# BIGBALLON/distribuuuu

Hardware: AMD Instinct MI355X
Metric: images/sec resnet50 train (whole node) (higher is better)
Workload: dtype bf16; 1 GPU; model=resnet50, global_batch=256, im_size=224, parallelism=dp1, syncbn=False, hipgraph=True

## Files before the change

### distribuuuu_amd/csrc/bind.cpp

```cpp
#include <torch/extension.h>

at::Tensor relu_fwd(at::Tensor x);
at::Tensor relu_bwd(at::Tensor gy, at::Tensor y);
at::Tensor add_relu_fwd(at::Tensor a, at::Tensor b);
at::Tensor se_scale_fwd(at::Tensor x, at::Tensor s);
at::Tensor dropout_fwd(at::Tensor x, double p, int64_t seed);
std::vector<at::Tensor> se_scale_bwd(at::Tensor gy, at::Tensor x,
                                     at::Tensor s);
std::vector<at::Tensor> bn_sums(at::Tensor x);
at::Tensor bn_reduce_partials(at::Tensor part);
std::vector<at::Tensor> bn_stats(at::Tensor x, at::Tensor gamma,
                                 at::Tensor beta,
                                 c10::optional<at::Tensor> rm_opt,
                                 c10::optional<at::Tensor> rv_opt,
                                 double momentum, double eps, bool training,
                                 c10::optional<at::Tensor> part_opt);
at::Tensor bn_apply_act(at::Tensor x, at::Tensor scale, at::Tensor shift,
                        int64_t act, c10::optional<at::Tensor> res);
at::Tensor bn_bwd_stats(at::Tensor gy, at::Tensor x,
                        c10::optional<at::Tensor> res, at::Tensor scale,
                        at::Tensor shift, int64_t act);
std::vector<at::Tensor> bn_bwd_apply(at::Tensor gy, at::Tensor x,
                                     c10::optional<at::Tensor> res,
                                     at::Tensor mean, at::Tensor rstd,
                                     at::Tensor gamma, at::Tensor scale,
                                     at::Tensor shift, at::Tensor sums,
                                     double total_count, int64_t act,
                                     bool training, bool need_gres);
std::vector<at::Tensor> bn_bwd(at::Tensor gy, at::Tensor x,
                               c10::optional<at::Tensor> res, at::Tensor mean,
                               at::Tensor rstd, at::Tensor gamma,
                               at::Tensor scale, at::Tensor shift,
                               int64_t act, bool training, bool need_gres,
                               c10::optional<at::Tensor> mask);
std::vector<at::Tensor> bn_apply_act_mask(at::Tensor x, at::Tensor scale,
                                          at::Tensor shift, int64_t act,
                                          at::Tensor res);
at::Tensor bn_apply_act_pad(at::Tensor x, at::Tensor scale, at::Tensor shift,
                            int64_t act, int64_t ph, int64_t pw);
std::vector<at::Tensor> bn_bwd_pad(at::Tensor gy, at::Tensor x,
                                   at::Tensor mean, at::Tensor rstd,
                                   at::Tensor gamma, at::Tensor scale,
                                   at::Tensor shift, int64_t act,
                                   bool training, int64_t ph, int64_t pw);
std::vector<at::Tensor> maxpool_fwd(at::Tensor x, int64_t K, int64_t S,
                                    int64_t P);
at::Tensor maxpool_bwd(at::Tensor gy, at::Tensor idx, int64_t H, int64_t W,
                       int64_t K, int64_t S, int64_t P);
at::Tensor gap_fwd(at::Tensor x);
at::Tensor gap_bwd(at::Tensor gy, int64_t H, int64_t W);
at::Tensor avgpool_fwd(at::Tensor x, int64_t K, int64_t S);
at::Tensor avgpool_bwd(at::Tensor gy, int64_t K, int64_t S, int64_t H,
                       int64_t W);
std::vector<at::Tensor> ce_fwd(at::Tensor logits, at::Tensor target);
at::Tensor ce_bwd(at::Tensor logits, at::Tensor target, at::Tensor lse,
                  at::Tensor gl);
std::vector<at::Tensor> topk_acc(at::Tensor logits, at::Tensor target,
                                 int64_t topk);
at::Tensor conv2d_fwd_v1(at::Tensor x, at::Tensor w, at::Tensor y,
                         int64_t Ho, int64_t Wo, int64_t sh, int64_t sw,
                         int64_t ph, int64_t pw, int64_t dh, int64_t dw,
                         int64_t groups);
at::Tensor conv2d_fwd(at::Tensor x, at::Tensor w, int64_t sh, int64_t sw,
                      int64_t ph, int64_t pw, int64_t dh, int64_t dw,
                      int64_t groups);
std::vector<at::Tensor> conv2d_fwd_bn(at::Tensor x, at::Tensor w, int64_t sh,
                                      int64_t sw, int64_t ph, int64_t pw,
                                      int64_t dh, int64_t dw, int64_t groups);
at::Tensor conv2d_dgrad(at::Tensor gy, at::Tensor w, int64_t H, int64_t W,
                        int64_t sh, int64_t sw, int64_t ph, int64_t pw,
                        int64_t dh, int64_t dw, int64_t groups);
std::vector<at::Tensor> conv2d_dgrad_bn(at::Tensor gy, at::Tensor w,
                                        int64_t H, int64_t W, int64_t sh,
                                        int64_t sw, int64_t ph, int64_t pw,
                                        int64_t dh, int64_t dw,
                                        int64_t groups, at::Tensor bnx,
                                        at::Tensor bnscale, at::Tensor bnshift,
                                        int64_t bnact);

std::tuple<at::Tensor, int64_t> conv2d_dgrad_acc(
    at::Tensor gy, at::Tensor w, int64_t H, int64_t W, int64_t sh, int64_t sw,
    int64_t ph, int64_t pw, int64_t dh, int64_t dw, int64_t groups,
    at::Tensor into, c10::optional<at::Tensor> pre_opt, int64_t pre_kind);

std::vector<at::Tensor> conv2d_dgrad_prep(at::Tensor w, int64_t Kt0,
                                          int64_t sh, int64_t sw, int64_t ph,
                                          int64_t pw, int64_t dh, int64_t dw,
                                          int64_t groups);

at::Tensor conv2d_dgrad_pre(at::Tensor gy, at::Tensor w, int64_t H,
                            int64_t W, int64_t sh, int64_t sw, int64_t ph,
                            int64_t pw, int64_t dh, int64_t dw,
                            int64_t groups, at::Tensor pre,
                            int64_t pre_kind);
at::Tensor gemm_nt(at::Tensor a, at::Tensor b);
at::Tensor conv2d_fwd_v2(at::Tensor x, at::Tensor w, int64_t sh, int64_t sw,
                         int64_t ph, int64_t pw, int64_t dh, int64_t dw);
at::Tensor weight_flip_t(at::Tensor w, int64_t groups);
at::Tensor dilate_nhwc(at::Tensor x, int64_t sh, int64_t sw);
at::Tensor pad_channels(at::Tensor x, int64_t Cn);
at::Tensor conv2d_wgrad(at::Tensor gy, at::Tensor x, int64_t R, int64_t S,
                        int64_t sh, int64_t sw, int64_t ph, int64_t pw,
                        int64_t dh, int64_t dw, int64_t groups);
at::Tensor dwconv_fwd(at::Tensor x, at::Tensor w, int64_t sh, int64_t sw,
                      int64_t ph, int64_t pw);
at::Tensor dwconv_dgrad(at::Tensor gy, at::Tensor w, int64_t H, int64_t W,
                        int64_t sh, int64_t sw, int64_t ph, int64_t pw);
at::Tensor dwconv_wgrad(at::Tensor gy, at::Tensor x, int64_t R, int64_t S,
                        int64_t sh, int64_t sw, int64_t ph, int64_t pw);
at::Tensor mhsa_fwd(at::Tensor q, at::Tensor k, at::Tensor vt, at::Tensor rw,
                    at::Tensor rh, int64_t H, int64_t W,
                    c10::optional<at::Tensor> pout, int64_t heads,
                    int64_t qpix, int64_t kpix, double scale);
std::vector<at::Tensor> mhsa_bwd(at::Tensor dO, at::Tensor P, at::Tensor q,
                                 at::Tensor kt, at::Tensor v,
                                 at::Tensor rel_w, at::Tensor rel_h,
                                 int64_t H, int64_t W, int64_t heads,
                                 int64_t qpix, int64_t kqoff, int64_t vpix,
                                 int64_t opix, double scale,
                                 at::Tensor dqk_out, at::Tensor dv_out);
at::Tensor mhsa_rel_tables(at::Tensor q, at::Tensor rel, int64_t rows,
                           int64_t heads, int64_t L, int64_t qpix,
                           double scale);
at::Tensor aug_crop_flip_norm(at::Tensor raw, at::Tensor meta, int64_t S,
                              std::vector<double> mean,
                              std::vector<double> std, at::ScalarType dtype);
void set_deterministic(bool on);
bool is_deterministic();
void sgd_step(at::Tensor table, double lr, double momentum,
              double dampening, double weight_decay, bool nesterov);

PYBIND11_MODULE(TORCH_EXTENSION_NAME, m) {
  m.def("relu_fwd", &relu_fwd);
  m.def("relu_bwd", &relu_bwd);
  m.def("add_relu_fwd", &add_relu_fwd);
  m.def("se_scale_fwd", &se_scale_fwd);
  m.def("dropout_fwd", &dropout_fwd);
  m.def("se_scale_bwd", &se_scale_bwd);
  m.def("bn_sums", &bn_sums);
  m.def("bn_reduce_partials", &bn_reduce_partials);
  m.def("bn_stats", &bn_stats, py::arg("x"), py::arg("gamma"), py::arg("beta"),
        py::arg("rm") = py::none(), py::arg("rv") = py::none(),
        py::arg("momentum") = 0.1, py::arg("eps") = 1e-5,
        py::arg("training") = true, py::arg("part") = py::none());
  m.def("bn_apply_act", &bn_apply_act, py::arg("x"), py::arg("scale"),
        py::arg("shift"), py::arg("act"), py::arg("res") = py::none());
  m.def("bn_apply_act_mask", &bn_apply_act_mask);
  m.def("bn_apply_act_pad", &bn_apply_act_pad);
  m.def("bn_bwd_pad", &bn_bwd_pad);
  m.def("bn_bwd_stats", &bn_bwd_stats, py::arg("gy"), py::arg("x"),
        py::arg("res"), py::arg("scale"), py::arg("shift"),
        py::arg("act"));
  m.def("bn_bwd_apply", &bn_bwd_apply, py::arg("gy"), py::arg("x"),
        py::arg("res"), py::arg("mean"), py::arg("rstd"),
        py::arg("gamma"), py::arg("scale"), py::arg("shift"), py::arg("sums"),
        py::arg("total_count"), py::arg("act"), py::arg("training"),
        py::arg("need_gres"));
  m.def("bn_bwd", &bn_bwd, py::arg("gy"), py::arg("x"),
        py::arg("res"), py::arg("mean"), py::arg("rstd"), py::arg("gamma"),
        py::arg("scale"), py::arg("shift"), py::arg("act"),
        py::arg("training"), py::arg("need_gres"),
        py::arg("mask") = py::none());
  m.def("maxpool_fwd", &maxpool_fwd);
  m.def("maxpool_bwd", &maxpool_bwd);
  m.def("gap_fwd", &gap_fwd);
  m.def("gap_bwd", &gap_bwd);
  m.def("avgpool_fwd", &avgpool_fwd);
  m.def("avgpool_bwd", &avgpool_bwd);
  m.def("ce_fwd", &ce_fwd);
  m.def("ce_bwd", &ce_bwd);
  m.def("topk_acc", &topk_acc);
  m.def("sgd_step", &sgd_step);
  m.def("conv2d_fwd", &conv2d_fwd);
  m.def("conv2d_fwd_v1", &conv2d_fwd_v1);
  m.def("conv2d_fwd_bn", &conv2d_fwd_bn);
  m.def("conv2d_dgrad", &conv2d_dgrad);
  m.def("conv2d_dgrad_bn", &conv2d_dgrad_bn);
  m.def("conv2d_dgrad_acc", &conv2d_dgrad_acc);
  m.def("conv2d_dgrad_prep", &conv2d_dgrad_prep);
  m.def("conv2d_dgrad_pre", &conv2d_dgrad_pre);
  m.def("conv2d_wgrad", &conv2d_wgrad);
  m.def("gemm_nt", &gemm_nt);
  m.def("conv2d_fwd_v2", &conv2d_fwd_v2);
  m.def("weight_flip_t", &weight_flip_t);
  m.def("dilate_nhwc", &dilate_nhwc);
  m.def("pad_channels", &pad_channels);
  m.def("dwconv_fwd", &dwconv_fwd);
  m.def("dwconv_dgrad", &dwconv_dgrad);
  m.def("dwconv_wgrad", &dwconv_wgrad);
  m.def("mhsa_fwd", &mhsa_fwd);
  m.def("mhsa_bwd", &mhsa_bwd);
  m.def("mhsa_rel_tables", &mhsa_rel_tables);
  m.def("aug_crop_flip_norm", &aug_crop_flip_norm);
  m.def("set_deterministic", &set_deterministic);
  m.def("is_deterministic", &is_deterministic);
}
```

### distribuuuu_amd/csrc/conv.hip

```cpp
#include "common.h"

static int v2_minrsc() {
  static const int v = []() {
    const char* e = getenv("DISTRIBUUUU_V2_MINRSC");
    return e ? atoi(e) : 512;
  }();
  return v;
}

static int v2_into_minrsc() {
  static const int v = []() {
    const char* e = getenv("DISTRIBUUUU_V2INTO_MINRSC");
    return e ? atoi(e) : v2_minrsc();
  }();
  return v;
}


typedef __attribute__((ext_vector_type(8))) short short8;
typedef __attribute__((ext_vector_type(4))) float f32x4;
typedef __bf16 bf16x8 __attribute__((ext_vector_type(8)));

namespace {

// ... 461 lines not shown
  int C, H, W;
  int R, S, SC;
  int sh, sw, ph, pw;
  int Ho, Wo;
  int RSC, RSCp;
  int64_t M;
  unsigned long long magicHoWo, magicWo, magicSC, magicC;
  float* part;
};

DEV_INLINE int magic_div2(int m, unsigned long long magic) {
  return (int)(((unsigned long long)(unsigned)m * magic) >> 47);
}

template <bool EMIT>
__global__ __launch_bounds__(256) void conv_smallk_kernel(SmallConvParams p) {
  __shared__ float slab4[4][16 * 68];
  const int tid = threadIdx.x, lane = tid & 63, wid = tid >> 6;
  const int il = lane & 15, kq = lane >> 4;
  const int64_t mbase = (int64_t)blockIdx.x * 256 + wid * 64;
  int pn[4], prow[4], pcol[4];
  bool mok[4];
#pragma unroll
  for (int mi = 0; mi < 4; ++mi) {
    const int64_t m = mbase + mi * 16 + il;
    mok[mi] = m < p.M;
    const int mm = (int)(mok[mi] ? m : 0);
    const int n = magic_div2(mm, p.magicHoWo);
    const int rem = mm - n * (p.Ho * p.Wo);
    const int ho = magic_div2(rem, p.magicWo);
    const int wo = rem - ho * p.Wo;
    pn[mi] = n;
    prow[mi] = ho * p.sh - p.ph;
    pcol[mi] = wo * p.sw - p.pw;
  }
  const __hip_bfloat16* wr[4];
#pragma unroll
  for (int ni = 0; ni < 4; ++ni)
    wr[ni] = p.w + (int64_t)(ni * 16 + il) * p.RSCp + kq * 8;
  f32x4 acc[4][4] = {};
  if (p.C % 32 == 0) {
    const int csteps = p.C / 32;
    for (int r = 0; r < p.R; ++r) {
#pragma unroll 1
      for (int sidx = 0; sidx < p.S; ++sidx) {
        const __hip_bfloat16* ab[4];
        bool ok[4];
#pragma unroll
        for (int mi = 0; mi < 4; ++mi) {
          const int h = prow[mi] + r;
          const int w_ = pcol[mi] + sidx;
          ok[mi] = mok[mi] && h >= 0 && h < p.H && w_ >= 0 && w_ < p.W;
          ab[mi] = p.x +
                   (((int64_t)pn[mi] * p.H + h) * p.W + w_) * p.C + kq * 8;
        }
        const int e0 = (r * p.S + sidx) * p.C;
        for (int cc = 0; cc < csteps; ++cc) {
          bf16x8 afrag[4], bfrag[4];
#pragma unroll
          for (int mi = 0; mi < 4; ++mi)
            afrag[mi] = ok[mi] ? *reinterpret_cast<const bf16x8*>(ab[mi] +
                                                                  cc * 32)
                               : bf16x8{};
#pragma unroll
          for (int ni = 0; ni < 4; ++ni)
            bfrag[ni] =
                *reinterpret_cast<const bf16x8*>(wr[ni] + e0 + cc * 32);
#pragma unroll
          for (int mi = 0; mi < 4; ++mi)
#pragma unroll
            for (int ni = 0; ni < 4; ++ni)
              acc[mi][ni] = __builtin_amdgcn_mfma_f32_16x16x32_bf16(
                  afrag[mi], bfrag[ni], acc[mi][ni], 0, 0, 0);
        }
      }
    }
  } else {
    const int ksteps = p.RSCp / 32;
    for (int t = 0; t < ksteps; ++t) {
      const int e = t * 32 + kq * 8;
      const int r = magic_div2(e, p.magicSC);
      const int rem2 = e - r * p.SC;
      const int sidx = magic_div2(rem2, p.magicC);
      const int c = rem2 - sidx * p.C;
      bf16x8 afrag[4], bfrag[4];
#pragma unroll
      for (int mi = 0; mi < 4; ++mi) {
        const int h = prow[mi] + r;
        const int w_ = pcol[mi] + sidx;
        const bool ok = mok[mi] && e < p.RSC && h >= 0 && h < p.H &&
                        w_ >= 0 && w_ < p.W;
        afrag[mi] =
            ok ? *reinterpret_cast<const bf16x8*>(
                     p.x + (((int64_t)pn[mi] * p.H + h) * p.W + w_) * p.C + c)
               : bf16x8{};
      }
#pragma unroll
      for (int ni = 0; ni < 4; ++ni)
        bfrag[ni] = *reinterpret_cast<const bf16x8*>(wr[ni] + t * 32);
#pragma unroll
      for (int mi = 0; mi < 4; ++mi)
#pragma unroll
        for (int ni = 0; ni < 4; ++ni)
          acc[mi][ni] = __builtin_amdgcn_mfma_f32_16x16x32_bf16(
              afrag[mi], bfrag[ni], acc[mi][ni], 0, 0, 0);
    }
  }
  float* slab = slab4[wid];
  const int er = lane >> 2, ec = (lane & 3) << 4;
  float ps = 0.f, pq = 0.f;
#pragma unroll
  for (int mi = 0; mi < 4; ++mi) {
#pragma unroll
    for (int ni = 0; ni < 4; ++ni)
#pragma unroll
      for (int rr = 0; rr < 4; ++rr)
        slab[(kq * 4 + rr) * 68 + ni * 16 + il] = acc[mi][ni][rr];
    __builtin_amdgcn_wave_barrier();
    const int64_t m = mbase + mi * 16 + er;
    if (m < p.M) {
      union {
        __hip_bfloat16 b[16];
        uint4 q[2];
      } u;
#pragma unroll
      for (int j = 0; j < 16; ++j)
        u.b[j] = from_f32<__hip_bfloat16>(slab[er * 68 + ec + j]);
      __hip_bfloat16* yp = p.y + m * 64 + ec;
      *reinterpret_cast<uint4*>(yp) = u.q[0];
      *reinterpret_cast<uint4*>(yp + 8) = u.q[1];
    }
    if (EMIT)
      bn_partial_col_accum(slab, ps, pq,
                           (int)min((int64_t)16, p.M - (mbase + mi * 16)),
                           lane);
    __builtin_amdgcn_wave_barrier();
  }
  if (EMIT) {
    __shared__ float xarea[3][2][64];
    if (wid > 0) {
      xarea[wid - 1][0][lane] = ps;
      xarea[wid - 1][1][lane] = pq;
    }
    __syncthreads();
    if (wid == 0) {
#pragma unroll
      for (int j = 0; j < 3; ++j) {
        ps += xarea[j][0][lane];
        pq += xarea[j][1][lane];
      }
      bn_partial_store(p.part, (int64_t)blockIdx.x * 128, 64, lane, 64, ps,
                       pq);
    }
  }
}


template <int CSTEPS, bool EMIT>
__global__ __launch_bounds__(256) void conv_smallk_pipe_kernel(
    SmallConvParams p) {
  __shared__ float slab4[4][16 * 68];
  const int tid = threadIdx.x, lane = tid & 63, wid = tid >> 6;
  const int il = lane & 15, kq = lane >> 4;
  const int64_t mbase = (int64_t)blockIdx.x * 256 + wid * 64;
  int pn[4], prow[4], pcol[4];
  bool mok[4];
#pragma unroll
  for (int mi = 0; mi < 4; ++mi) {
    const int64_t m = mbase + mi * 16 + il;
    mok[mi] = m < p.M;
    const int mm = (int)(mok[mi] ? m : 0);
    const int n = magic_div2(mm, p.magicHoWo);
    const int rem = mm - n * (p.Ho * p.Wo);
    const int ho = magic_div2(rem, p.magicWo);
    const int wo = rem - ho * p.Wo;
    pn[mi] = n;
    prow[mi] = ho * p.sh - p.ph;
    pcol[mi] = wo * p.sw - p.pw;
  }
  const __hip_bfloat16* wr[4];
#pragma unroll
  for (int ni = 0; ni < 4; ++ni)
    wr[ni] = p.w + (int64_t)(ni * 16 + il) * p.RSCp + kq * 8;
  const int S = p.S;
  const int steps = p.R * S * CSTEPS;
  int r = 0, si = 0, cc = 0;
  bf16x8 Af[2][4], Bf[2][4];
  auto issue = [&](int buf) {
#pragma unroll
    for (int mi = 0; mi < 4; ++mi) {
      const int h = prow[mi] + r;
      const int w_ = pcol[mi] + si;
      const bool ok = mok[mi] && h >= 0 && h < p.H && w_ >= 0 && w_ < p.W;
      const __hip_bfloat16* ap =
          ok ? p.x + (((int64_t)pn[mi] * p.H + h) * p.W + w_) * p.C +
                   cc * 32 + kq * 8
             : p.zbuf;
      Af[buf][mi] = *reinterpret_cast<const bf16x8*>(ap);
    }
    const int e0 = (r * S + si) * p.C + cc * 32;
#pragma unroll
    for (int ni = 0; ni < 4; ++ni)
      Bf[buf][ni] = *reinterpret_cast<const bf16x8*>(wr[ni] + e0);
    ++cc;
    if (cc == CSTEPS) {
      cc = 0;
      ++si;
      if (si == S) {
        si = 0;
        ++r;
      }
    }
  };
  f32x4 acc[4][4] = {};
  issue(0);
  for (int i = 0; i < steps; i += 2) {
    if (i + 1 < steps) issue(1);
#pragma unroll
    for (int mi = 0; mi < 4; ++mi)
#pragma unroll
      for (int ni = 0; ni < 4; ++ni)
        acc[mi][ni] = __builtin_amdgcn_mfma_f32_16x16x32_bf16(
            Af[0][mi], Bf[0][ni], acc[mi][ni], 0, 0, 0);
    if (i + 1 < steps) {
      if (i + 2 < steps) issue(0);
#pragma unroll
      for (int mi = 0; mi < 4; ++mi)
#pragma unroll
        for (int ni = 0; ni < 4; ++ni)
          acc[mi][ni] = __builtin_amdgcn_mfma_f32_16x16x32_bf16(
              Af[1][mi], Bf[1][ni], acc[mi][ni], 0, 0, 0);
    }
  }
  float* slab = slab4[wid];
  const int er = lane >> 2, ec = (lane & 3) << 4;
  float ps = 0.f, pq = 0.f;
#pragma unroll
  for (int mi = 0; mi < 4; ++mi) {
#pragma unroll
    for (int ni = 0; ni < 4; ++ni)
#pragma unroll
      for (int rr = 0; rr < 4; ++rr)
        slab[(kq * 4 + rr) * 68 + ni * 16 + il] = acc[mi][ni][rr];
    __builtin_amdgcn_wave_barrier();
    const int64_t m = mbase + mi * 16 + er;
    if (m < p.M) {
      union {
        __hip_bfloat16 b[16];
        uint4 q[2];
      } u;
#pragma unroll
      for (int j = 0; j < 16; ++j)
        u.b[j] = from_f32<__hip_bfloat16>(slab[er * 68 + ec + j]);
      __hip_bfloat16* yp = p.y + m * 64 + ec;
      *reinterpret_cast<uint4*>(yp) = u.q[0];
      *reinterpret_cast<uint4*>(yp + 8) = u.q[1];
    }
    if (EMIT)
      bn_partial_col_accum(slab, ps, pq,
                           (int)min((int64_t)16, p.M - (mbase + mi * 16)),
                           lane);
    __builtin_amdgcn_wave_barrier();
  }
  if (EMIT) {
    __shared__ float xarea[3][2][64];
    if (wid > 0) {
      xarea[wid - 1][0][lane] = ps;
      xarea[wid - 1][1][lane] = pq;
    }
    __syncthreads();
    if (wid == 0) {
#pragma unroll
      for (int j = 0; j < 3; ++j) {
        ps += xarea[j][0][lane];
        pq += xarea[j][1][lane];
      }
      bn_partial_store(p.part, (int64_t)blockIdx.x * 128, 64, lane, 64, ps,
                       pq);
    }
  }
}

}

at::Tensor conv2d_fwd_into_fp32(at::Tensor x, at::Tensor w, at::Tensor y,
                                int64_t Ho, int64_t Wo, int64_t sh, int64_t sw,
                                int64_t ph, int64_t pw, int64_t dh, int64_t dw,
                                int64_t groups, int64_t osh, int64_t osw,
                                int64_t oh0, int64_t ow0,
                                at::Tensor* part_out);

struct BnBwdEmit {
  const __hip_bfloat16* x;
  const float* scale;
  const float* shift;
  int act;
};

at::Tensor conv2d_fwd_v2_into(at::Tensor x, at::Tensor w, at::Tensor y,
                              int64_t Ho, int64_t Wo, int64_t groups,
                              int64_t osh, int64_t osw, int64_t oh0,
                              int64_t ow0, bool acc = false);

at::Tensor conv2d_fwd_into(at::Tensor x, at::Tensor w, at::Tensor y, int64_t Ho,
                           int64_t Wo, int64_t sh, int64_t sw, int64_t ph,
                           int64_t pw, int64_t dh, int64_t dw, int64_t groups,
                           int64_t osh = 1, int64_t osw = 1, int64_t oh0 = 0,
                           int64_t ow0 = 0, at::Tensor* part_out = nullptr,
                           const BnBwdEmit* bemit = nullptr,
                           bool acc = false) {
  CHECK_GPU(x);
  if (x.scalar_type() == at::kFloat)
    return conv2d_fwd_into_fp32(x, w, y, Ho, Wo, sh, sw, ph, pw, dh, dw,
                                groups, osh, osw, oh0, ow0,
                                bemit ? nullptr : part_out);
  TORCH_CHECK(x.scalar_type() == at::kBFloat16, "conv2d_fwd: bf16/fp32 only");
  {
    static const bool v2i_off = []() {
      const char* e = getenv("DISTRIBUUUU_CONV_V2INTO");
      return e && e[0] == '0';
    }();
    const int Cgi = w.size(1), Ri = w.size(2), Si = w.size(3);
    const int Kgi = (int)(w.size(0) / groups);
    if (!v2i_off && part_out == nullptr && bemit == nullptr && ph == 0 &&
        pw == 0 && sh == 1 && sw == 1 && dh == 1 && dw == 1 &&
        (Si * Cgi) % 64 == 0 && Kgi >= 96 &&
        (int64_t)Ri * Si * Cgi >= v2_into_minrsc() && Cgi % 8 == 0 &&
        Ho + Ri - 1 <= x.size(2) && Wo + Si - 1 <= x.size(3))
      return conv2d_fwd_v2_into(x, w, y, Ho, Wo, groups, osh, osw, oh0, ow0,
                                acc);
  }
  check_nhwc(x, "x");
  check_nhwc(w, "w");
  const int N = x.size(0), Ct = x.size(1), H = x.size(2), W = x.size(3);
  const int Kt = w.size(0), Cg = w.size(1), R = w.size(2), S = w.size(3);
  TORCH_CHECK(Ct == Cg * groups, "channel/group mismatch");
  TORCH_CHECK(Cg % 8 == 0, "conv2d_fwd: per-group C must be a multiple of 8");
  const int Kg = Kt / groups;
  ConvParams p;
  p.x = (const __hip_bfloat16*)x.data_ptr();
  p.w = (const __hip_bfloat16*)w.data_ptr();
  p.y = (__hip_bfloat16*)y.data_ptr();
  p.N = N; p.H = H; p.W = W; p.Ct = Ct; p.Kt = Kt;
  p.R = R; p.S = S; p.Cg = Cg; p.Kg = Kg;
  p.sh = sh; p.sw = sw; p.ph = ph; p.pw = pw; p.dh = dh; p.dw = dw;
  p.Ho = Ho; p.Wo = Wo;
  p.HoA = y.size(2); p.WoA = y.size(3);
  p.osh = osh; p.osw = osw;
  p.oh0 = oh0; p.ow0 = ow0;
  p.M = N * Ho * Wo;
  p.nspan = (S * Cg + BK - 1) / BK;
  p.ksteps = R * p.nspan;
  p.tiles_m = (p.M + BM - 1) / BM;
  p.part = nullptr;
  p.bnx = nullptr;
  p.bnscale = nullptr;
  p.bnshift = nullptr;
  p.bnact = 0;
  dim3 grid(p.tiles_m, (Kg + BN - 1) / BN, groups);
  if (bemit != nullptr) {
    *part_out = at::empty({(int64_t)p.tiles_m, (int64_t)2 * Kt},
                          x.options().dtype(at::kFloat));
    p.part = part_out->data_ptr<float>();
    p.bnx = bemit->x;
    p.bnscale = bemit->scale;
    p.bnshift = bemit->shift;
    p.bnact = bemit->act;
    hipLaunchKernelGGL(conv_igemm_fwd_kernel<2>, grid, dim3(256), 0,
                       cur_stream(), p);
  } else if (part_out != nullptr) {
    *part_out = at::empty({(int64_t)p.tiles_m, (int64_t)2 * Kt},
                          x.options().dtype(at::kFloat));
    p.part = part_out->data_ptr<float>();
    hipLaunchKernelGGL(conv_igemm_fwd_kernel<1>, grid, dim3(256), 0,
                       cur_stream(), p);
  } else if (acc) {
    hipLaunchKernelGGL((conv_igemm_fwd_kernel<0, true>), grid, dim3(256), 0,
                       cur_stream(), p);
  } else {
    hipLaunchKernelGGL(conv_igemm_fwd_kernel<0>, grid, dim3(256), 0,
                       cur_stream(), p);
  }
  return y;
}

at::Tensor conv2d_fwd_v2p(at::Tensor x, at::Tensor w, int64_t sh, int64_t sw,
                          int64_t ph, int64_t pw, int64_t dh, int64_t dw,
                          int64_t groups, at::Tensor* part_out,
                          const BnBwdEmit* bemit = nullptr);
at::Tensor conv2d_fwd_v2_flat(at::Tensor x, at::Tensor wp, int64_t Kt_,
                              int64_t Cg_, int64_t R_, int64_t S_, int64_t sh,
                              int64_t sw, int64_t ph, int64_t pw, int64_t dh,
                              int64_t dw, int64_t groups,
                              at::Tensor* part_out, const BnBwdEmit* bemit,
                              at::Tensor* acc_into = nullptr);

static at::Tensor conv2d_fwd_impl(at::Tensor x, at::Tensor w, int64_t sh,
                                  int64_t sw, int64_t ph, int64_t pw,
                                  int64_t dh, int64_t dw, int64_t groups,
                                  at::Tensor* part_out,
                                  const BnBwdEmit* bemit = nullptr) {
  const int N = x.size(0), H = x.size(2), W = x.size(3);
  const int Kt = w.size(0), R = w.size(2), S = w.size(3);
  static const bool v2_off = []() {
    const char* e = getenv("DISTRIBUUUU_CONV_V2");
    return e && e[0] == '0';
  }();
  const int C_ = x.size(1);
  const int v2Kg = Kt / (int)groups;
  const int v2Cg = C_ / (int)groups;
  static const int v2_mink = []() {
    const char* e = getenv("DISTRIBUUUU_V2_MINK");
    return e ? atoi(e) : 192;
  }();
  if (!v2_off && v2Kg >= v2_mink &&
      (int64_t)R * S * v2Cg >= v2_minrsc() &&
      v2Cg % 8 == 0 && x.scalar_type() == at::kBFloat16)
    return conv2d_fwd_v2p(x, w, sh, sw, ph, pw, dh, dw, groups, part_out,
                          bemit);
  static const bool small_off = []() {
    const char* e = getenv("DISTRIBUUUU_CONV_SMALL");
    return e && e[0] == '0';
  }();
  if (!small_off && groups == 1 && R == 1 && S == 1 && sh == 1 && sw == 1 &&
      C_ % 32 == 0 && Kt % 64 == 0 && x.scalar_type() == at::kBFloat16 &&
      ((C_ <= 64 && Kt <= 512) || (C_ <= 256 && Kt <= 64))) {
    const int64_t M = (int64_t)N * H * W;
    auto y = at::empty({N, Kt, H, W},
                       x.options().memory_format(at::MemoryFormat::ChannelsLast));
    SmallGemmParams sp;
    sp.x = (const __hip_bfloat16*)x.data_ptr();
    sp.w = (const __hip_bfloat16*)w.data_ptr();
    sp.y = (__hip_bfloat16*)y.data_ptr();
    sp.C = C_; sp.Kt = Kt; sp.M = M;
    sp.part = nullptr;
    const dim3 sg((int)((M + 255) / 256));
    if (bemit != nullptr) part_out = nullptr;
    if (part_out != nullptr) {
      *part_out = at::empty({(int64_t)sg.x, (int64_t)2 * Kt},
                            x.options().dtype(at::kFloat));
      sp.part = part_out->data_ptr<float>();
      if (C_ == 64)
        hipLaunchKernelGGL((conv_gemm_smallc_kernel<2, true>), sg, dim3(256),
                           0, cur_stream(), sp);
      else if (C_ == 32)
        hipLaunchKernelGGL((conv_gemm_smallc_kernel<1, true>), sg, dim3(256),
                           0, cur_stream(), sp);
      else
        hipLaunchKernelGGL(conv_gemm_small_kernel<true>, sg, dim3(256), 0,
                           cur_stream(), sp);
    } else if (C_ == 64)
      hipLaunchKernelGGL((conv_gemm_smallc_kernel<2, false>), sg, dim3(256),
                         0, cur_stream(), sp);
    else if (C_ == 32)
      hipLaunchKernelGGL((conv_gemm_smallc_kernel<1, false>), sg, dim3(256),
                         0, cur_stream(), sp);
    else
      hipLaunchKernelGGL(conv_gemm_small_kernel<false>, sg, dim3(256), 0,
                         cur_stream(), sp);
    return y;
  }
  const int Ho = (H + 2 * ph - dh * (R - 1) - 1) / sh + 1;
  const int Wo = (W + 2 * pw - dw * (S - 1) - 1) / sw + 1;
  if (!small_off && groups == 1 && Kt == 64 && C_ <= 64 && C_ % 8 == 0 &&
      dh == 1 && dw == 1 && R * S > 1 && R * S * C_ <= 1024 &&
      x.scalar_type() == at::kBFloat16) {
    const int RSC = R * S * C_;
    const int RSCp = (RSC + 31) / 32 * 32;
    at::Tensor wsp = w;
    if (RSCp != RSC) {
      wsp = at::zeros({(int64_t)Kt, RSCp}, w.options());
      wsp.narrow(1, 0, RSC).copy_(
          w.permute({0, 2, 3, 1}).reshape({(int64_t)Kt, RSC}));
    }
    auto y = at::empty({N, Kt, Ho, Wo},
                       x.options().memory_format(at::MemoryFormat::ChannelsLast));
    SmallConvParams sp;
    sp.x = (const __hip_bfloat16*)x.data_ptr();
    sp.w = (const __hip_bfloat16*)wsp.data_ptr();
    sp.y = (__hip_bfloat16*)y.data_ptr();
    sp.C = C_; sp.H = H; sp.W = W;
    sp.R = R; sp.S = S; sp.SC = S * C_;
    sp.sh = sh; sp.sw = sw; sp.ph = ph; sp.pw = pw;
    sp.Ho = Ho; sp.Wo = Wo;
    sp.RSC = RSC; sp.RSCp = RSCp;
    sp.M = (int64_t)N * Ho * Wo;
    sp.magicHoWo = ((1ULL << 47) / ((unsigned long long)Ho * Wo)) + 1;
    sp.magicWo = ((1ULL << 47) / (unsigned long long)Wo) + 1;
    sp.magicSC = ((1ULL << 47) / (unsigned long long)(S * C_)) + 1;
    sp.magicC = ((1ULL << 47) / (unsigned long long)C_) + 1;
    static at::Tensor zbuf;
    if (!zbuf.defined() || zbuf.device() != x.device())
      zbuf = at::zeros({8}, x.options());
    sp.zbuf = (const __hip_bfloat16*)zbuf.data_ptr();
    sp.part = nullptr;
    const dim3 skg((int)((sp.M + 255) / 256));
    if (bemit != nullptr) part_out = nullptr;
    if (part_out != nullptr) {
      *part_out = at::empty({(int64_t)skg.x, 128},
                            x.options().dtype(at::kFloat));
      sp.part = part_out->data_ptr<float>();
      if (C_ == 64)
        hipLaunchKernelGGL((conv_smallk_pipe_kernel<2, true>), skg, dim3(256),
                           0, cur_stream(), sp);
      else if (C_ == 32)
        hipLaunchKernelGGL((conv_smallk_pipe_kernel<1, true>), skg, dim3(256),
                           0, cur_stream(), sp);
      else
        hipLaunchKernelGGL(conv_smallk_kernel<true>, skg, dim3(256), 0,
                           cur_stream(), sp);
    } else if (C_ == 64)
      hipLaunchKernelGGL((conv_smallk_pipe_kernel<2, false>), skg, dim3(256),
                         0, cur_stream(), sp);
    else if (C_ == 32)
      hipLaunchKernelGGL((conv_smallk_pipe_kernel<1, false>), skg, dim3(256),
                         0, cur_stream(), sp);
    else
      hipLaunchKernelGGL(conv_smallk_kernel<false>, skg, dim3(256), 0,
                         cur_stream(), sp);
    return y;
  }
  auto y = at::empty({N, Kt, Ho, Wo},
                     x.options().memory_format(at::MemoryFormat::ChannelsLast));
  return conv2d_fwd_into(x, w, y, Ho, Wo, sh, sw, ph, pw, dh, dw, groups, 1,
                         1, 0, 0, part_out, bemit);
}


at::Tensor conv2d_fwd_v1(at::Tensor x, at::Tensor w, at::Tensor y,
                         int64_t Ho, int64_t Wo, int64_t sh, int64_t sw,
                         int64_t ph, int64_t pw, int64_t dh, int64_t dw,
                         int64_t groups) {
  return conv2d_fwd_into(x, w, y, Ho, Wo, sh, sw, ph, pw, dh, dw, groups);
}

at::Tensor conv2d_fwd(at::Tensor x, at::Tensor w, int64_t sh, int64_t sw,
                      int64_t ph, int64_t pw, int64_t dh, int64_t dw,
                      int64_t groups) {
  return conv2d_fwd_impl(x, w, sh, sw, ph, pw, dh, dw, groups, nullptr);
}

std::vector<at::Tensor> conv2d_fwd_bn(at::Tensor x, at::Tensor w, int64_t sh,
                                      int64_t sw, int64_t ph, int64_t pw,
                                      int64_t dh, int64_t dw, int64_t groups) {
  at::Tensor part;
  auto y = conv2d_fwd_impl(x, w, sh, sw, ph, pw, dh, dw, groups, &part);
  TORCH_CHECK(part.defined(), "conv2d_fwd_bn: dispatch path without partials");
  return {y, part};
}

at::Tensor gemm_nt(at::Tensor a, at::Tensor b) {
  TORCH_CHECK(a.dim() == 2 && b.dim() == 2, "gemm_nt expects 2-D");
  const int M = a.size(0), K = a.size(1), Nc = b.size(0);
  auto a_cl = a.reshape({M, K, 1, 1}).contiguous(at::MemoryFormat::ChannelsLast);
  auto b_cl = b.reshape({Nc, K, 1, 1}).contiguous(at::MemoryFormat::ChannelsLast);
  auto y = conv2d_fwd(a_cl, b_cl, 1, 1, 0, 0, 1, 1, 1);
  return y.reshape({M, Nc});
}

namespace {

template <typename T>
__global__ void weight_flip_t_kernel(const T* __restrict__ w, T* __restrict__ wt,
                                     int Kg, int Cg, int R, int S, int G) {
  const int64_t total = (int64_t)G * Cg * R * S * Kg;
  for (int64_t i = (int64_t)blockIdx.x * blockDim.x + threadIdx.x; i < total;
       i += (int64_t)gridDim.x * blockDim.x) {
    int64_t t = i;
    const int k = t % Kg;
    t /= Kg;
    const int s = t % S;
    t /= S;
    const int r = t % R;
    t /= R;
    const int c = t % Cg;
    const int g = t / Cg;
    wt[i] = w[((((int64_t)(g * Kg + k) * R) + (R - 1 - r)) * S + (S - 1 - s)) *
                  Cg +
              c];
  }
}

template <typename T>
__global__ void dilate_nhwc_kernel(const T* __restrict__ x, T* __restrict__ y,
                                   int N, int Ho, int Wo, int C, int sh,
                                   int sw, int Hd, int Wd) {
  const int64_t total = (int64_t)N * Ho * Wo * C;
  for (int64_t i = (int64_t)blockIdx.x * blockDim.x + threadIdx.x; i < total;
       i += (int64_t)gridDim.x * blockDim.x) {
    const int c = i % C;
    int64_t t = i / C;
    const int wo = t % Wo;
    t /= Wo;
    const int ho = t % Ho;
    const int n = t / Ho;
    y[(((int64_t)n * Hd + ho * sh) * Wd + wo * sw) * C + c] = x[i];
  }
}

}

namespace {
template <typename T>
__global__ void weight_flip_t_span_kernel(const T* __restrict__ w,
                                          T* __restrict__ o, int Kg, int Cg,
                                          int R, int S, int G, int SPAN64) {
  const int64_t total = (int64_t)G * Cg * R * SPAN64;
  const int SKg = S * Kg;
  for (int64_t i = (int64_t)blockIdx.x * blockDim.x + threadIdx.x; i < total;
       i += (int64_t)gridDim.x * blockDim.x) {
    const int sp = i % SPAN64;
    int64_t t = i / SPAN64;
    const int r = t % R;
    t /= R;
    const int c = t % Cg;
    const int g = t / Cg;
    T v = from_f32<T>(0.f);
    if (sp < SKg) {
      const int sidx = sp / Kg;
      const int k = sp - sidx * Kg;
      v = w[((((int64_t)(g * Kg + k) * R) + (R - 1 - r)) * S +
             (S - 1 - sidx)) * Cg + c];
    }
    o[i] = v;
  }
}
}

at::Tensor weight_flip_t_span(at::Tensor w, int64_t groups, int64_t SPAN64) {
  CHECK_GPU(w);
  check_nhwc(w, "w");
  const int Kt = w.size(0), Cg = w.size(1), R = w.size(2), S = w.size(3);
  const int Kg = Kt / groups;
  auto o = at::empty({(int64_t)Cg * groups * R * SPAN64}, w.options());
  const int64_t total = o.numel();
  DISPATCH_FLOAT_AND_BF16(w.scalar_type(), "weight_flip_t_span", [&] {
    hipLaunchKernelGGL((weight_flip_t_span_kernel<scalar_t>),
                       dim3(grid_1d(total, 256)), dim3(256), 0, cur_stream(),
                       (const scalar_t*)w.data_ptr(), (scalar_t*)o.data_ptr(),
                       Kg, Cg, R, S, (int)groups, (int)SPAN64);
  });
  return o;
}

at::Tensor weight_flip_t(at::Tensor w, int64_t groups) {
  CHECK_GPU(w);
  check_nhwc(w, "w");
  const int Kt = w.size(0), Cg = w.size(1), R = w.size(2), S = w.size(3);
  const int Kg = Kt / groups;
  auto wt = at::empty({Cg * groups, Kg, R, S},
                      w.options().memory_format(at::MemoryFormat::ChannelsLast));
  int64_t total = (int64_t)Kt * Cg * R * S;
  DISPATCH_FLOAT_AND_BF16(w.scalar_type(), "weight_flip_t", [&] {
    hipLaunchKernelGGL((weight_flip_t_kernel<scalar_t>),
                       dim3(grid_1d(total, 256)), dim3(256), 0, cur_stream(),
                       (const scalar_t*)w.data_ptr(), (scalar_t*)wt.data_ptr(),
                       Kg, Cg, R, S, (int)groups);
  });
  return wt;
}

at::Tensor dilate_nhwc(at::Tensor x, int64_t sh, int64_t sw) {
  CHECK_GPU(x);
  check_nhwc(x, "x");
  const int N = x.size(0), C = x.size(1), Ho = x.size(2), Wo = x.size(3);
  const int Hd = (Ho - 1) * sh + 1, Wd = (Wo - 1) * sw + 1;
  auto y = at::empty({N, C, Hd, Wd},
                     x.options().memory_format(at::MemoryFormat::ChannelsLast));
  y.zero_();
  int64_t total = (int64_t)N * Ho * Wo * C;
  DISPATCH_FLOAT_AND_BF16(x.scalar_type(), "dilate_nhwc", [&] {
    hipLaunchKernelGGL((dilate_nhwc_kernel<scalar_t>),
                       dim3(grid_1d(total, 256)), dim3(256), 0, cur_stream(),
                       (const scalar_t*)x.data_ptr(), (scalar_t*)y.data_ptr(),
                       N, Ho, Wo, C, sh, sw, Hd, Wd);
  });
  return y;
}

namespace {
template <typename T>
__global__ void pad_channels_kernel(const T* __restrict__ x, T* __restrict__ y,
                                    int64_t rows, int C, int Cn) {
  constexpr int V = 16 / sizeof(T);
  if (Cn == V) {
    union {
      T b[V];
      uint4 q;
    } u;
    for (int64_t r = (int64_t)blockIdx.x * blockDim.x + threadIdx.x;
         r < rows; r += (int64_t)gridDim.x * blockDim.x) {
#pragma unroll
      for (int j = 0; j < V; ++j)
        u.b[j] = j < C ? x[r * C + j] : from_f32<T>(0.f);
      *reinterpret_cast<uint4*>(y + r * V) = u.q;
    }
    return;
  }
  const int64_t total = rows * Cn;
  for (int64_t i = (int64_t)blockIdx.x * blockDim.x + threadIdx.x; i < total;
       i += (int64_t)gridDim.x * blockDim.x) {
    const int c = i % Cn;
    const int64_t r = i / Cn;
    y[i] = (c < C) ? x[r * C + c] : from_f32<T>(0.f);
  }
}
}

at::Tensor pad_channels(at::Tensor x, int64_t Cn) {
  CHECK_GPU(x);
  check_nhwc(x, "x");
  const int N = x.size(0), C = x.size(1), H = x.size(2), W = x.size(3);
  auto y = at::empty({N, Cn, H, W},
                     x.options().memory_format(at::MemoryFormat::ChannelsLast));
  const int64_t rows = (int64_t)N * H * W;
  DISPATCH_FLOAT_AND_BF16(x.scalar_type(), "pad_channels", [&] {
    hipLaunchKernelGGL((pad_channels_kernel<scalar_t>),
                       dim3(grid_1d(rows * Cn, 256)), dim3(256), 0,
                       cur_stream(), (const scalar_t*)x.data_ptr(),
                       (scalar_t*)y.data_ptr(), rows, C, (int)Cn);
  });
  return y;
}

static at::Tensor conv2d_dgrad_impl(at::Tensor gy, at::Tensor w, int64_t H,
                                    int64_t W, int64_t sh, int64_t sw,
                                    int64_t ph, int64_t pw, int64_t dh,
                                    int64_t dw, int64_t groups,
                                    at::Tensor* part_out,
                                    const BnBwdEmit* bemit,
                                    const at::Tensor* pre = nullptr,
                                    int64_t pre_kind = -1) {
  CHECK_GPU(gy);
  check_nhwc(gy, "gy");
  const int N = gy.size(0);
  const int Cg = w.size(1), R = w.size(2), S = w.size(3);
  const int Ct = Cg * groups;
  {
    const int Kt0 = gy.size(1);
    const int dKg0 = Ct / (int)groups;
    const int dCg0 = Kt0 / (int)groups;
    static const int v2mink2 = []() {
      const char* e = getenv("DISTRIBUUUU_V2_MINK");
      return e ? atoi(e) : 192;
    }();
    static const bool v2off2 = []() {
      const char* e = getenv("DISTRIBUUUU_CONV_V2");
      return e && e[0] == '0';
    }();
    if (sh == 1 && sw == 1 && dh * (R - 1) >= ph &&
        dw * (S - 1) >= pw && Kt0 % (8 * (int)groups) == 0 && !v2off2 &&
        dKg0 >= v2mink2 && (int64_t)R * S * dCg0 >= v2_minrsc() &&
        dCg0 % 8 == 0 &&
        gy.scalar_type() == at::kBFloat16) {
      const int SPAN64 = ((int)(S * dCg0) + 63) / 64 * 64;
      auto wsp = (pre != nullptr && pre_kind == 1)
                     ? *pre
                     : weight_flip_t_span(w, groups, SPAN64);
      return conv2d_fwd_v2_flat(gy, wsp, Ct, dCg0, R, S, 1, 1,
                                dh * (R - 1) - ph, dw * (S - 1) - pw, dh, dw,
                                groups, part_out, bemit);
    }
  }
  auto wt = (pre != nullptr && pre_kind == 0)
                ? *pre
                : weight_flip_t(w, groups);
  if (R == 1 && S == 1 && (sh > 1 || sw > 1) && ph == 0 && pw == 0) {
    auto gx1 = at::empty({N, Ct, H, W}, gy.options().memory_format(
                                            at::MemoryFormat::ChannelsLast));
    gx1.zero_();
    conv2d_fwd_into(gy, wt, gx1, gy.size(2), gy.size(3), 1, 1, 0, 0, 1, 1,
                    groups, sh, sw, 0, 0, part_out, bemit);
    return gx1;
  }
  if (R == 3 && S == 3 && sh == 2 && sw == 2 && dh == 1 && dw == 1 &&
      ph == 1 && pw == 1) {
    auto gx = at::empty({N, Ct, H, W}, gy.options().memory_format(
                                           at::MemoryFormat::ChannelsLast));
    std::vector<at::Tensor> parts;
    for (int h0 = 0; h0 < 2; ++h0) {
      const int64_t hu = (H - h0 + 1) >> 1;
      auto wr = (h0 == 0) ? wt.slice(2, 1, 2) : wt.slice(2, 0, 3, 2);
      for (int w0 = 0; w0 < 2; ++w0) {
        const int64_t wu = (W - w0 + 1) >> 1;
        auto wsub = ((w0 == 0) ? wr.slice(3, 1, 2) : wr.slice(3, 0, 3, 2))
                        .contiguous(at::MemoryFormat::ChannelsLast);
        at::Tensor sub_part;
        conv2d_fwd_into(gy, wsub, gx, hu, wu, 1, 1, 0, 0, 1, 1, groups, 2, 2,
                        h0, w0, bemit ? &sub_part : nullptr, bemit);
        if (bemit && sub_part.defined()) parts.push_back(sub_part);
      }
    }
    if (bemit && part_out && parts.size() == 4)
      *part_out = at::cat(parts, 0);
    return gx;
  }
  const int Kt_ = gy.size(1);
  if (sh == 1 && sw == 1 && dh * (R - 1) >= ph && dw * (S - 1) >= pw &&
      (R > 1 || (ph == 0 && pw == 0)) &&
      (groups == 1 || Kt_ % (8 * groups) == 0)) {
    return conv2d_fwd_impl(gy, wt, 1, 1, dh * (R - 1) - ph,
                           dw * (S - 1) - pw, dh, dw, groups, part_out,
                           bemit);
  }
  (void)Kt_;
  auto gyd = (sh == 1 && sw == 1) ? gy : dilate_nhwc(gy, sh, sw);
  const int Hd = gyd.size(2), Wd = gyd.size(3);
  const int pph = dh * (R - 1) - ph, ppw = dw * (S - 1) - pw;
  TORCH_CHECK(pph >= 0 && ppw >= 0, "dgrad pad underflow");
  (void)Hd; (void)Wd;
  auto gx = at::empty({N, Ct, H, W}, gy.options().memory_format(
                                           at::MemoryFormat::ChannelsLast));
  conv2d_fwd_into(gyd, wt, gx, H, W, 1, 1, pph, ppw, dh, dw, groups, 1, 1, 0,
                  0, part_out, bemit);
  return gx;
}

at::Tensor conv2d_dgrad(at::Tensor gy, at::Tensor w, int64_t H, int64_t W,
                        int64_t sh, int64_t sw, int64_t ph, int64_t pw,
                        int64_t dh, int64_t dw, int64_t groups) {
  return conv2d_dgrad_impl(gy, w, H, W, sh, sw, ph, pw, dh, dw, groups,
                           nullptr, nullptr);
}

std::vector<at::Tensor> conv2d_dgrad_prep(at::Tensor w, int64_t Kt0,
                                          int64_t sh, int64_t sw, int64_t ph,
                                          int64_t pw, int64_t dh, int64_t dw,
                                          int64_t groups) {
  const int Cg = w.size(1), R = w.size(2), S = w.size(3);
  const int Ct = Cg * (int)groups;
  const int dKg0 = Ct / (int)groups;
  const int dCg0 = (int)(Kt0 / groups);
  static const int v2mink4 = []() {
    const char* e = getenv("DISTRIBUUUU_V2_MINK");
    return e ? atoi(e) : 192;
  }();
// ... 125 lines not shown
```

Before: 8529 images/sec.

## Add dedicated pointwise 1x1 conv kernel with register-resident activations

Adds a specialized MFMA kernel for 1x1 stride-1 bf16 convolutions. It keeps the full input-channel slice of each activation row in registers and streams weight chunks of 64 output channels through LDS. The kernel has epilogue variants that emit BatchNorm partial sums or accumulate into an existing output. The kernel is routed automatically for C=128→512 and C=256→1024 expansions, and for the residual-accumulate case, to cut redundant activation reloads versus the generic conv path. The risks are lower occupancy from heavy register use and a different BN-partial reduction order.

```diff
diff --git a/distribuuuu_amd/csrc/bind.cpp b/distribuuuu_amd/csrc/bind.cpp
--- a/distribuuuu_amd/csrc/bind.cpp
+++ b/distribuuuu_amd/csrc/bind.cpp
@@ -61,6 +61,20 @@
                          int64_t Ho, int64_t Wo, int64_t sh, int64_t sw,
                          int64_t ph, int64_t pw, int64_t dh, int64_t dw,
                          int64_t groups);
+std::vector<at::Tensor> conv2d_fwd_v1_bn(at::Tensor x, at::Tensor w,
+                                         at::Tensor y, int64_t Ho, int64_t Wo,
+                                         int64_t sh, int64_t sw, int64_t ph,
+                                         int64_t pw, int64_t dh, int64_t dw,
+                                         int64_t groups);
+at::Tensor conv2d_fwd_v1_acc(at::Tensor x, at::Tensor w, at::Tensor y,
+                             int64_t Ho, int64_t Wo, int64_t sh, int64_t sw,
+                             int64_t ph, int64_t pw, int64_t dh, int64_t dw,
+                             int64_t groups);
+at::Tensor conv2d_pw(at::Tensor x, at::Tensor w, int64_t ksplit);
+std::vector<at::Tensor> conv2d_pw_bn(at::Tensor x, at::Tensor w,
+                                     int64_t ksplit);
+at::Tensor conv2d_pw_acc(at::Tensor x, at::Tensor w, at::Tensor into,
+                         int64_t ksplit);
 at::Tensor conv2d_fwd(at::Tensor x, at::Tensor w, int64_t sh, int64_t sw,
                       int64_t ph, int64_t pw, int64_t dh, int64_t dw,
                       int64_t groups);
@@ -173,6 +187,14 @@
   m.def("sgd_step", &sgd_step);
   m.def("conv2d_fwd", &conv2d_fwd);
   m.def("conv2d_fwd_v1", &conv2d_fwd_v1);
+  m.def("conv2d_fwd_v1_bn", &conv2d_fwd_v1_bn);
+  m.def("conv2d_fwd_v1_acc", &conv2d_fwd_v1_acc);
+  m.def("conv2d_pw", &conv2d_pw, py::arg("x"), py::arg("w"),
+        py::arg("ksplit") = 0);
+  m.def("conv2d_pw_bn", &conv2d_pw_bn, py::arg("x"), py::arg("w"),
+        py::arg("ksplit") = 0);
+  m.def("conv2d_pw_acc", &conv2d_pw_acc, py::arg("x"), py::arg("w"),
+        py::arg("into"), py::arg("ksplit") = 0);
   m.def("conv2d_fwd_bn", &conv2d_fwd_bn);
   m.def("conv2d_dgrad", &conv2d_dgrad);
   m.def("conv2d_dgrad_bn", &conv2d_dgrad_bn);
diff --git a/distribuuuu_amd/csrc/conv.hip b/distribuuuu_amd/csrc/conv.hip
--- a/distribuuuu_amd/csrc/conv.hip
+++ b/distribuuuu_amd/csrc/conv.hip
@@ -787,19 +787,47 @@
                               int64_t osh, int64_t osw, int64_t oh0,
                               int64_t ow0, bool acc = false);
 
+bool conv_pw_supports(int64_t C, int64_t Kt, bool with_part);
+at::Tensor conv_pw_into(at::Tensor x, at::Tensor w, at::Tensor y,
+                        at::Tensor* part_out, bool acc, int64_t ksplit);
+
+static bool pw_route(const at::Tensor& x, const at::Tensor& w, int64_t sh,
+                     int64_t sw, int64_t ph, int64_t pw, int64_t groups,
+                     bool with_part, bool acc) {
+  static const bool pw_off = []() {
+    const char* e = getenv("DISTRIBUUUU_CONV_PW");
+    return e && e[0] == '0';
+  }();
+  if (pw_off || groups != 1 || w.size(2) != 1 || w.size(3) != 1 || sh != 1 ||
+      sw != 1 || ph != 0 || pw != 0 || x.scalar_type() != at::kBFloat16 ||
+      w.scalar_type() != at::kBFloat16)
+    return false;
+  const int64_t C = x.size(1), Kt = w.size(0);
+  if (!conv_pw_supports(C, Kt, with_part)) return false;
+  if (acc)
+    return C == 128 && (Kt == 256 || Kt == 512);
+  return (C == 128 && Kt == 512) || (C == 256 && Kt == 1024);
+}
+
 at::Tensor conv2d_fwd_into(at::Tensor x, at::Tensor w, at::Tensor y, int64_t Ho,
                            int64_t Wo, int64_t sh, int64_t sw, int64_t ph,
                            int64_t pw, int64_t dh, int64_t dw, int64_t groups,
                            int64_t osh = 1, int64_t osw = 1, int64_t oh0 = 0,
                            int64_t ow0 = 0, at::Tensor* part_out = nullptr,
                            const BnBwdEmit* bemit = nullptr,
-                           bool acc = false) {
+                           bool acc = false, bool allow_pw = true) {
   CHECK_GPU(x);
   if (x.scalar_type() == at::kFloat)
     return conv2d_fwd_into_fp32(x, w, y, Ho, Wo, sh, sw, ph, pw, dh, dw,
                                 groups, osh, osw, oh0, ow0,
                                 bemit ? nullptr : part_out);
   TORCH_CHECK(x.scalar_type() == at::kBFloat16, "conv2d_fwd: bf16/fp32 only");
+  if (allow_pw && acc && part_out == nullptr && bemit == nullptr &&
+      osh == 1 && osw == 1 && oh0 == 0 && ow0 == 0 && Ho == x.size(2) &&
+      Wo == x.size(3) && y.size(2) == Ho && y.size(3) == Wo &&
+      y.size(1) == w.size(0) && y.scalar_type() == at::kBFloat16 &&
+      pw_route(x, w, sh, sw, ph, pw, groups, false, true))
+    return conv_pw_into(x, w, y, nullptr, true, 0);
   {
     static const bool v2i_off = []() {
       const char* e = getenv("DISTRIBUUUU_CONV_V2INTO");
@@ -945,6 +973,12 @@
                          cur_stream(), sp);
     return y;
   }
+  if (bemit == nullptr &&
+      pw_route(x, w, sh, sw, ph, pw, groups, part_out != nullptr, false)) {
+    auto y = at::empty({N, Kt, H, W},
+                       x.options().memory_format(at::MemoryFormat::ChannelsLast));
+    return conv_pw_into(x, w, y, part_out, false, 0);
+  }
   const int Ho = (H + 2 * ph - dh * (R - 1) - 1) / sh + 1;
   const int Wo = (W + 2 * pw - dw * (S - 1) - 1) / sw + 1;
   if (!small_off && groups == 1 && Kt == 64 && C_ <= 64 && C_ % 8 == 0 &&
@@ -1016,7 +1050,47 @@
                          int64_t Ho, int64_t Wo, int64_t sh, int64_t sw,
                          int64_t ph, int64_t pw, int64_t dh, int64_t dw,
                          int64_t groups) {
-  return conv2d_fwd_into(x, w, y, Ho, Wo, sh, sw, ph, pw, dh, dw, groups);
+  return conv2d_fwd_into(x, w, y, Ho, Wo, sh, sw, ph, pw, dh, dw, groups, 1,
+                         1, 0, 0, nullptr, nullptr, false, false);
+}
+
+std::vector<at::Tensor> conv2d_fwd_v1_bn(at::Tensor x, at::Tensor w,
+                                         at::Tensor y, int64_t Ho, int64_t Wo,
+                                         int64_t sh, int64_t sw, int64_t ph,
+                                         int64_t pw, int64_t dh, int64_t dw,
+                                         int64_t groups) {
+  at::Tensor part;
+  conv2d_fwd_into(x, w, y, Ho, Wo, sh, sw, ph, pw, dh, dw, groups, 1, 1, 0, 0,
+                  &part, nullptr, false, false);
+  return {y, part};
+}
+
+at::Tensor conv2d_fwd_v1_acc(at::Tensor x, at::Tensor w, at::Tensor y,
+                             int64_t Ho, int64_t Wo, int64_t sh, int64_t sw,
+                             int64_t ph, int64_t pw, int64_t dh, int64_t dw,
+                             int64_t groups) {
+  return conv2d_fwd_into(x, w, y, Ho, Wo, sh, sw, ph, pw, dh, dw, groups, 1,
+                         1, 0, 0, nullptr, nullptr, true, false);
+}
+
+at::Tensor conv2d_pw(at::Tensor x, at::Tensor w, int64_t ksplit) {
+  auto y = at::empty({x.size(0), w.size(0), x.size(2), x.size(3)},
+                     x.options().memory_format(at::MemoryFormat::ChannelsLast));
+  return conv_pw_into(x, w, y, nullptr, false, ksplit);
+}
+
+std::vector<at::Tensor> conv2d_pw_bn(at::Tensor x, at::Tensor w,
+                                     int64_t ksplit) {
+  auto y = at::empty({x.size(0), w.size(0), x.size(2), x.size(3)},
+                     x.options().memory_format(at::MemoryFormat::ChannelsLast));
+  at::Tensor part;
+  conv_pw_into(x, w, y, &part, false, ksplit);
+  return {y, part};
+}
+
+at::Tensor conv2d_pw_acc(at::Tensor x, at::Tensor w, at::Tensor into,
+                         int64_t ksplit) {
+  return conv_pw_into(x, w, into, nullptr, true, ksplit);
 }
 
 at::Tensor conv2d_fwd(at::Tensor x, at::Tensor w, int64_t sh, int64_t sw,
diff --git a/distribuuuu_amd/csrc/conv_pw.hip b/distribuuuu_amd/csrc/conv_pw.hip
--- /dev/null
+++ b/distribuuuu_amd/csrc/conv_pw.hip
@@ -0,0 +1,247 @@
+#include "common.h"
+
+typedef __attribute__((ext_vector_type(4))) float f32x4;
+typedef __bf16 bf16x8 __attribute__((ext_vector_type(8)));
+
+namespace {
+
+struct PwParams {
+  const __hip_bfloat16* x;
+  const __hip_bfloat16* w;
+  __hip_bfloat16* y;
+  int C, Kt;
+  int64_t M;
+  float* part;
+};
+
+DEV_INLINE void lds_barrier() {
+  asm volatile("s_waitcnt lgkmcnt(0)" ::: "memory");
+  __builtin_amdgcn_s_barrier();
+  asm volatile("" ::: "memory");
+}
+
+template <int CS, int EPI>
+__global__ __launch_bounds__(256, 2) void conv_pw_kernel(PwParams p) {
+  constexpr int NI = CS >= 5 ? 2 : 4;
+  constexpr int BROWS = NI == 4 ? 256 : 128;
+  constexpr int RS = CS * 32 + 8;
+  __shared__ __align__(16) __hip_bfloat16 ldsB[64 * RS];
+  __shared__ float slab4[4][16 * 68];
+  __shared__ float xarea[EPI == 1 ? 4 * 2 * 64 : 4];
+  const int tid = threadIdx.x, lane = tid & 63;
+  const int wid = __builtin_amdgcn_readfirstlane(tid >> 6);
+  const int wr = NI == 4 ? wid : wid >> 1;
+  const int wc = NI == 4 ? 0 : wid & 1;
+  const int il = lane & 15, kq = lane >> 4;
+  const int64_t mbase = (int64_t)blockIdx.x * BROWS + wr * 64;
+  float* slab = slab4[wid];
+
+  bf16x8 afr[CS][4];
+#pragma unroll
+  for (int mi = 0; mi < 4; ++mi) {
+    const int64_t m = mbase + mi * 16 + il;
+    const __hip_bfloat16* xr = p.x + (m < p.M ? m : 0) * p.C + kq * 8;
+#pragma unroll
+    for (int cs = 0; cs < CS; ++cs)
+      afr[cs][mi] = m < p.M ? *reinterpret_cast<const bf16x8*>(xr + cs * 32)
+                            : bf16x8{};
+  }
+
+  bf16x8 stg[CS];
+  auto bgload = [&](int c) {
+#pragma unroll
+    for (int j = 0; j < CS; ++j) {
+      const int q = tid + j * 256;
+      stg[j] = *reinterpret_cast<const bf16x8*>(
+          p.w + ((int64_t)c * 64 + q / (4 * CS)) * p.C + (q % (4 * CS)) * 8);
+    }
+  };
+  auto bswrite = [&]() {
+#pragma unroll
+    for (int j = 0; j < CS; ++j) {
+      const int q = tid + j * 256;
+      *reinterpret_cast<bf16x8*>(
+          &ldsB[(q / (4 * CS)) * RS + (q % (4 * CS)) * 8]) = stg[j];
+    }
+  };
+
+  const int cstride = gridDim.y;
+  const int nown = ((p.Kt >> 6) - (int)blockIdx.y + cstride - 1) / cstride;
+  auto chunk_of = [&](int t) { return (int)blockIdx.y + t * cstride; };
+  if (nown > 0) {
+    bgload(chunk_of(0));
+    bswrite();
+  }
+  lds_barrier();
+
+  constexpr int NQ = NI / 2;
+  const int er = lane >> 2;
+  const int ec = (lane & 3) * (NQ * 8);
+  const unsigned yoff = er * p.Kt + ec + wc * 32;
+  union Pack {
+    __hip_bfloat16 b[NQ * 8];
+    uint4 q[NQ];
+  };
+  constexpr bool OLDPF = CS < 7;
+  Pack oldc[EPI == 2 ? 4 : 1];
+  auto oldload = [&](int mi, int c) {
+    if (mbase + mi * 16 + er < p.M) {
+      const __hip_bfloat16* yp =
+          p.y + (mbase + mi * 16) * p.Kt + c * 64 + yoff;
+#pragma unroll
+      for (int h = 0; h < NQ; ++h)
+        oldc[mi].q[h] = *reinterpret_cast<const uint4*>(yp + h * 8);
+    }
+  };
+  if (EPI == 2 && OLDPF && nown > 0) {
+#pragma unroll
+    for (int mi = 0; mi < 4; ++mi) oldload(mi, chunk_of(0));
+  }
+
+  for (int t = 0; t < nown; ++t) {
+    const int k0 = chunk_of(t) << 6;
+    const bool more = t + 1 < nown;
+    const int chn = chunk_of(more ? t + 1 : t);
+    f32x4 acc[4][NI] = {};
+#pragma unroll
+    for (int cs = 0; cs < CS; ++cs) {
+      bf16x8 bfrag[NI];
+#pragma unroll
+      for (int ni = 0; ni < NI; ++ni)
+        bfrag[ni] = *reinterpret_cast<const bf16x8*>(
+            &ldsB[((wc * NI + ni) * 16 + il) * RS + cs * 32 + kq * 8]);
+#pragma unroll
+      for (int mi = 0; mi < 4; ++mi)
+#pragma unroll
+        for (int ni = 0; ni < NI; ++ni)
+          acc[mi][ni] = __builtin_amdgcn_mfma_f32_16x16x32_bf16(
+              afr[cs][mi], bfrag[ni], acc[mi][ni], 0, 0, 0);
+    }
+    lds_barrier();
+    if (more) bgload(chn);
+    float ps = 0.f, pq = 0.f;
+#pragma unroll
+    for (int mi = 0; mi < 4; ++mi) {
+      const int64_t m0 = mbase + mi * 16;
+#pragma unroll
+      for (int ni = 0; ni < NI; ++ni)
+#pragma unroll
+        for (int rr = 0; rr < 4; ++rr)
+          slab[(kq * 4 + rr) * 68 + ni * 16 + il] = acc[mi][ni][rr];
+      __builtin_amdgcn_wave_barrier();
+      if (EPI == 2 && !OLDPF) oldload(mi, chunk_of(t));
+      if (m0 + er < p.M) {
+        Pack u;
+#pragma unroll
+        for (int j = 0; j < NQ * 8; ++j) {
+          float v = slab[er * 68 + ec + j];
+          if (EPI == 2)
+            v = to_f32(from_f32<__hip_bfloat16>(v)) +
+                to_f32(oldc[mi].b[j]);
+          u.b[j] = from_f32<__hip_bfloat16>(v);
+        }
+        if (EPI == 2 && OLDPF && more) oldload(mi, chn);
+        __hip_bfloat16* yp = p.y + m0 * p.Kt + k0 + yoff;
+#pragma unroll
+        for (int h = 0; h < NQ; ++h)
+          *reinterpret_cast<uint4*>(yp + h * 8) = u.q[h];
+      }
+      if (EPI == 1)
+        bn_partial_col_accum(slab, ps, pq,
+                             (int)min((int64_t)16, p.M - m0), lane);
+      __builtin_amdgcn_wave_barrier();
+    }
+    if (EPI == 1) {
+      xarea[(wid * 2 + 0) * 64 + lane] = ps;
+      xarea[(wid * 2 + 1) * 64 + lane] = pq;
+    }
+    if (more) bswrite();
+    lds_barrier();
+    constexpr int PSTEP = NI == 4 ? 1 : 2;
+    if (EPI == 1 && (NI == 4 ? (wid & 1) == 0 : wid < 2) &&
+        lane < NI * 16) {
+      const int64_t prow =
+          NI == 4 ? (int64_t)blockIdx.x * 2 + (wid >> 1) : (int64_t)blockIdx.x;
+      if (prow * 128 < p.M) {
+        float* pr = p.part + prow * 2 * p.Kt + k0 + wc * 32 + lane;
+        pr[0] = xarea[(wid * 2 + 0) * 64 + lane] +
+                xarea[((wid + PSTEP) * 2 + 0) * 64 + lane];
+        pr[p.Kt] = xarea[(wid * 2 + 1) * 64 + lane] +
+                   xarea[((wid + PSTEP) * 2 + 1) * 64 + lane];
+      }
+    }
+  }
+}
+
+template <int EPI>
+void pw_launch_epi(int cs, dim3 grid, const PwParams& p) {
+#define PW_CASE(N)                                                       \
+  case N:                                                                \
+    hipLaunchKernelGGL((conv_pw_kernel<N, EPI>), grid, dim3(256), 0,     \
+                       cur_stream(), p);                                 \
+    break;
+  switch (cs) {
+    PW_CASE(3) PW_CASE(4) PW_CASE(5) PW_CASE(6) PW_CASE(7) PW_CASE(8)
+    default:
+      TORCH_CHECK(false, "conv_pw: unsupported C ", cs * 32);
+  }
+#undef PW_CASE
+}
+
+}
+
+bool conv_pw_supports(int64_t C, int64_t Kt, bool with_part) {
+  (void)with_part;
+  return C > 64 && C <= 256 && C % 32 == 0 && Kt >= 128 && Kt % 64 == 0;
+}
+
+at::Tensor conv_pw_into(at::Tensor x, at::Tensor w, at::Tensor y,
+                        at::Tensor* part_out, bool acc, int64_t ksplit) {
+  CHECK_GPU(x);
+  check_nhwc(x, "x");
+  check_nhwc(w, "w");
+  check_nhwc(y, "y");
+  TORCH_CHECK(x.scalar_type() == at::kBFloat16 &&
+                  w.scalar_type() == at::kBFloat16 &&
+                  y.scalar_type() == at::kBFloat16,
+              "conv_pw: bf16 only");
+  const int64_t N = x.size(0), C = x.size(1), H = x.size(2), W = x.size(3);
+  const int64_t Kt = w.size(0);
+  TORCH_CHECK(w.size(1) == C && w.size(2) == 1 && w.size(3) == 1,
+              "conv_pw: w must be [Kt, C, 1, 1]");
+  TORCH_CHECK(!(acc && part_out != nullptr), "conv_pw: ACC has no partials");
+  TORCH_CHECK(conv_pw_supports(C, Kt, part_out != nullptr),
+              "conv_pw: unsupported shape C=", C, " Kt=", Kt);
+  TORCH_CHECK(y.size(0) == N && y.size(1) == Kt && y.size(2) == H &&
+                  y.size(3) == W,
+              "conv_pw: y must be [N, Kt, H, W]");
+  PwParams p;
+  p.x = (const __hip_bfloat16*)x.data_ptr();
+  p.w = (const __hip_bfloat16*)w.data_ptr();
+  p.y = (__hip_bfloat16*)y.data_ptr();
+  p.C = (int)C; p.Kt = (int)Kt; p.M = N * H * W;
+  p.part = nullptr;
+  const int64_t tiles_m = ceil_div(p.M, C >= 160 ? 128 : 256);
+  const int nchunk = (int)(Kt / 64);
+  int ks = (int)ksplit;
+  if (ks <= 0) {
+    const int64_t want =
+        (int64_t)at::cuda::getCurrentDeviceProperties()->multiProcessorCount;
+    ks = 1;
+    while (tiles_m * ks < want && nchunk >= 4 * ks) ks *= 2;
+  }
+  TORCH_CHECK(ks <= nchunk, "conv_pw: ksplit ", ks, " too large for Kt=",
+              Kt);
+  const dim3 grid((unsigned)tiles_m, (unsigned)ks);
+  if (part_out != nullptr) {
+    *part_out = at::empty({ceil_div(p.M, 128), 2 * Kt},
+                          x.options().dtype(at::kFloat));
+    p.part = part_out->data_ptr<float>();
+    pw_launch_epi<1>((int)(C / 32), grid, p);
+  } else if (acc) {
+    pw_launch_epi<2>((int)(C / 32), grid, p);
+  } else {
+    pw_launch_epi<0>((int)(C / 32), grid, p);
+  }
+  return y;
+}
```

New measurement: 8529 images/sec. No clear change (-0.0%).
